# SerezD/vqvae-vqgan-pytorch-lightning

Hardware: AMD Instinct MI355X
Metric: images/sec/node (256x256 bs=32/GPU) VQ-VAE train step (higher is better)
Workload: dtype bf16; 1 GPU; standard_vqvae cb=1024, 256x256 bs=32/GPU (encoder+VQ+decoder fwd/bwd + AdamW); yaml=example_confs/standard_vqvae.yaml, global_batch=32, parallelism=dp1, launch=hipGraph replay (fwd+bwd) + eager all-reduce + AdamW, deterministic=False

## Files before the change

include/vqk.h:

```cpp
#ifndef VQK_H_
#define VQK_H_

#include <stddef.h>
#include <stdint.h>

#ifdef __cplusplus
extern "C" {
#endif

#define VQK_F32 0
#define VQK_BF16 1

enum vqk_status {
    VQK_OK = 0,
    VQK_ERR_SHAPE = -1,
    VQK_ERR_DTYPE = -2,
    VQK_ERR_ALIGN = -3,
    VQK_ERR_LAUNCH = -4,
    VQK_ERR_ARG = -5,
    VQK_ERR_WORKSPACE = -6
};

const char* vqk_status_str(int status);
int vqk_version(void);
// ... 145 lines not shown
                               float scale, const void* zeros, void* stream);
int vqk_conv2d_wgrad_pooled_dy_phase(int dtype, const void* x, const void* dy_pooled, float* dw, int n, int h, int w, int cin,
                                     int cout, float scale, const void* zeros, void* stream);
int vqk_conv2d_wgrad_general(int dtype, const void* x, const void* dy, float* dw, int n, int h_in, int w_in, int cin,
                             int cout, int ksize, int stride, int pad, int mode, int h_out, int w_out,
                             const void* zeros, void* stream);
int vqk_conv2d_fprop_x3_gnstats(const float* x, const void* w5, const float* bias, const float* residual, float* y, int n, int h_in,
                                int w_in, int cin, int cout, int ups, double* gn_ws, int groups, const void* zeros, void* stream);
int vqk_split_pair_f32(const float* src, void* dst, int64_t rows, int c, void* stream);
int vqk_conv2d_wgrad_x3_f32(const float* x, const float* dy, float* dw, int n, int h_in, int w_in, int cin, int cout, int ups,
                            float scale, void* stream);
int vqk_conv2d_wgrad_x3(const void* x_pair, const void* dy_pair, float* dw, int n, int h_in, int w_in, int cin, int cout, int ups,
                        float scale, const void* zeros, void* stream);
int vqk_conv2d_wgrad_general_scaled(int dtype, const void* x, const void* dy, float* dw, int n, int h_in, int w_in, int cin,
                                    int cout, int ksize, int stride, int pad, int mode, int h_out, int w_out, float scale,
                                    const void* zeros, void* stream);
int vqk_conv2d_s2_supported(int dtype, int n, int h_out, int w_out, int cin, int cout, int backward);
int vqk_conv2d_s2_fprop(int dtype, const void* x, const void* wq, const float* bias, void* y, int n, int h_out, int w_out,
                        int cin, int cout, int act, float acc_scale, float out_gain, const void* zeros, void* stream);
int vqk_conv2d_s2_dgrad(int dtype, const void* dy, const void* w3, const void* wt0, void* dx, int n, int h_out, int w_out,
                        int cin, int cout, float acc_scale, const void* zeros, void* stream);
int vqk_conv_weight_layout(int dtype, int n, int h_in, int w_in, int cin, int cout, int ksize, int ups);
int64_t vqk_conv_packed_elems(int cout, int cin, int ksize, int layout);
int vqk_conv_pack_weights(const float* w, void* out, int dtype, int cout, int cin, int ksize, int transpose,
                          int layout, void* stream);
int vqk_conv_pack_multi(const int64_t* descs_dev, int ndesc, int blocks_per_desc, void* stream);
int vqk_conv_set_variant(int variant);
int vqk_conv_fprop_plan(int dtype, int out_dtype, int n, int h_in, int w_in, int cin, int cout, int ksize, int ups, int act,
                        int wlayout, int flags, int* details);
const char* vqk_conv_fprop_form_name(int form, int dtype);
int vqk_set_deterministic(int on, void* ws, int64_t ws_bytes);
int vqk_set_scratch(void* ws, int64_t ws_bytes);
int vqk_set_tile_queue(void* ws, int64_t ws_bytes);
typedef struct vqk_ctx vqk_ctx;
int vqk_ctx_create(vqk_ctx** ctx);
int vqk_ctx_destroy(vqk_ctx* ctx);
int vqk_ctx_make_current(vqk_ctx* ctx);
int vqk_ctx_set_scratch(vqk_ctx* ctx, void* ws, int64_t ws_bytes);
int vqk_ctx_set_tile_queue(vqk_ctx* ctx, void* ws, int64_t ws_bytes);
int vqk_ctx_set_deterministic(vqk_ctx* ctx, int on, void* ws, int64_t ws_bytes);
int vqk_set_tuning(const char* name, int value);
int vqk_reset_tuning(void);
int vqk_tuning_count(void);
const char* vqk_tuning_name(int i);
int vqk_conv_set_block_caps(int stream_blocks, int wgrad_blocks);
int vqk_probe_stream_add(const float* src, float* dst, int64_t bytes, int blocks, int passes, int sleep, void* stream);
int vqk_calib_fill(void* w, int64_t bytes, void* stream);
int vqk_calib_mfma(const void* w, int64_t w_bytes, float* sink, int iters, int blocks, void* stream);
int64_t vqk_calib_mfma_flops(int iters, int blocks);
int vqk_calib_copy(const void* src, void* dst, int64_t bytes, void* stream);
int vqk_conv_pack_dgrad(const float* w, void* wt, int dtype, int cout, int cin, int ksize, void* stream);
int vqk_conv2d_wgrad(int dtype, const void* x, const void* dy, float* dw, int n, int h_in, int w_in, int cin,
                     int cout, int ksize, int ups, const void* zeros, void* stream);
typedef struct vqk_wgrad_item {
    const void* x;
    const void* dy;
    float* dw;
    int dtype, n, h, w, cin, cout, ksize, ups;
    float scale;
    int reserved;
} vqk_wgrad_item;
int vqk_conv3x3_wgrad_group(const vqk_wgrad_item* items, int n_items, const void* zeros, void* stream);
int vqk_conv3x3_wgrad_group_plan(const vqk_wgrad_item* items, int n_items, int* splits, int* launches);
int64_t vqk_conv2d_wgrad_edge_ws_bytes(void);
int vqk_conv2d_wgrad_edge(int dtype, const void* x, const void* dy, float* dw, void* ws, int64_t ws_bytes, int n, int h,
                          int w, int cin, int cout, const void* zeros, void* stream);
int vqk_conv2d_wgrad_edge_true(int dtype, const void* x, const void* dy, float* dw, void* ws, int64_t ws_bytes, int n, int h,
                               int w, int cin, int cout, int thin_true, const void* zeros, void* stream);
int vqk_conv2d_thin_out(int dtype, const void* x, const void* w, const float* bias, void* y, int n, int h, int wd, int cin,
                        int cout, int act, const void* zeros, void* stream);
int vqk_colsum(int dtype, const void* x, int64_t rows, int c, float* out, void* stream);
int vqk_colsum_lead(int dtype, const void* x, int64_t rows, int c, int c_out, float scale, float* out, void* stream);
int vqk_cast(const float* src, void* dst, int dtype, int64_t n, void* stream);

int vqk_gn_stats(int dtype, const void* x, int n, int64_t hw, int c, int groups, float eps,
                 double* acc, float* stats, void* stream);
int vqk_gn_apply(int dtype, const void* x, const float* stats, const float* w, const float* b, void* y,
                 int n, int64_t hw, int c, int groups, int silu, void* stream);
int vqk_gn_forward(int dtype, const void* x, const float* w, const float* b, void* y, float* stats, double* ws, int n,
                   int64_t hw, int c, int groups, float eps, int silu, void* stream);
int vqk_gn_forward_presummed(int dtype, const void* x, const float* w, const float* b, void* y, float* stats, double* ws,
                             int n, int64_t hw, int c, int groups, float eps, int silu, void* stream);
int vqk_gn_forward_presummed_parts(int dtype, const void* x, const float* w, const float* b, void* y, float* stats,
                                   const double* parts, int nblk, double* sums, int n, int64_t hw, int c, int groups, float eps,
                                   int silu, void* stream);
int vqk_gn_backward(int dtype, const void* x, const float* stats, const float* w, const float* b, const void* dy,
                    void* dx, float* dw, float* db, double* red, int n, int64_t hw, int c, int groups, int silu,
                    int accumulate, const void* add, void* stream);
int vqk_gn_backward_ws(int dtype, const void* x, const float* stats, const float* w, const float* b, const void* dy,
                       void* dx, float* dw, float* db, double* red, int64_t ws_doubles, int n, int h, int wd, int c, int groups,
                       int silu, int accumulate, const void* add, const void* add_pooled, float add_scale, void* stream);
int vqk_gn_cluster_timeouts(int* count);
int vqk_gn_backward_colsum(int dtype, const void* x, const float* stats, const float* w, const float* b, const void* dy,
                           void* dx, float* dw, float* db, double* red, int64_t ws_doubles, int n, int h, int wd, int c, int groups,
                           int silu, int accumulate, const void* add, float* dx_colsum, void* stream);
int vqk_gn_backward_pooled_add(int dtype, const void* x, const float* stats, const float* w, const float* b, const void* dy,
                               void* dx, float* dw, float* db, double* red, int n, int h, int wd, int c, int groups, int silu,
                               const void* add_pooled, float add_scale, void* stream);

int vqk_pool2x2(int dtype, const void* x, void* y, int n, int h, int w, int c, float scale, void* stream);
int vqk_unpool2x2(int dtype, const void* x, void* y, int n, int h, int w, int c, float scale, void* stream);
int vqk_preprocess(const float* images, void* x_pad, int dtype, float* target, int n, int h, int w, int cpad,
                   void* stream);
int vqk_augment_preprocess(const float* images, const float* box, const int32_t* flip, void* x_pad, int dtype, float* target,
                           int n, int h, int w, int cpad, void* stream);
int vqk_sse(int dtype, const void* recon, const float* target, int64_t n, float* loss, void* stream);
// ... 124 lines not shown
```

vqvae-vqgan-pytorch-lightning_amd/_native.py:

```python
from __future__ import annotations

import ctypes
import fcntl
import os
import subprocess
from ctypes import c_char_p, c_double, c_float, c_int, c_int32, c_int64, c_void_p, POINTER

_HERE = os.path.dirname(os.path.abspath(__file__))
_CSRC = os.path.join(_HERE, 'csrc')
_SO = os.environ.get('VQK_LIB') or os.path.join(_HERE, 'libvqk.so')
_lib = None

P = c_void_p
I, L, F = c_int, c_int64, c_float


class WgradItem(ctypes.Structure):
    _fields_ = [('x', c_void_p), ('dy', c_void_p), ('dw', c_void_p), ('dtype', c_int), ('n', c_int), ('h', c_int), ('w', c_int),
                ('cin', c_int), ('cout', c_int), ('ksize', c_int), ('ups', c_int), ('scale', c_float), ('reserved', c_int)]


_PROTOS = {
    'vqk_row_sqnorm_f32': [P, L, I, P, P],
    'vqk_vq_assign_f32': [P, P, P, P, L, I, I, I, P, P],
# ... 34 lines not shown
    'vqk_conv4x4_bgrad': [I, P, P, L, I, I, F, I, P, L, P],
    'vqk_bn_forward': [I, P, P, P, P, P, P, P, P, P, L, I, F, F, I, I, P, L, P],
    'vqk_bn_backward': [I, P, P, P, P, P, P, P, P, P, I, L, I, I, P, L, P],
    'vqk_rvq_forward_f32': [P, P, P, L, L, I, I, I, P, P, P, P, P, P],
    'vqk_rvq_decode_f32': [P, P, L, I, I, I, P, P, P],
    'vqk_rvq_backward_f32': [P, P, P, P, I, L, I, I, I, F, F, P, P, P, P, L, P],
    'vqk_l2norm_rows_f32': [P, L, I, P, P, P],
    'vqk_cos_prepare_f32': [P, I, I, P, L, P],
    'vqk_cos_forward_f32': [P, P, L, L, I, I, P, P, P, P, P, P],
    'vqk_cos_sse_f32': [P, P, L, I, P, P],
    'vqk_cos_decode_f32': [P, P, L, L, I, I, P, P, P],
    'vqk_cos_backward_f32': [P, P, P, P, I, L, I, I, F, F, P, P, P, P, L, P],
    'vqk_gvq_forward_f32': [P, P, P, L, I, I, I, P, P, P, P, P, P],
    'vqk_gvq_decode_f32': [P, P, L, I, I, I, P, P, P],
    'vqk_gvq_backward_f32': [P, P, P, P, I, L, I, I, I, F, F, P, P, P, P, L, P],
    'vqk_simvq_project_f32': [P, P, P, I, I, P, P],
    'vqk_simvq_hist_i32': [P, L, I, P, P],
    'vqk_simvq_backward_f32': [P, P, P, P, P, I, L, I, I, F, F, P, P, P, P, P, L, P],
    'vqk_kmeans_seed_step_f32': [P, L, I, I, I, P, P, P, P, P, L, P],
    'vqk_kmeans_update_f32': [P, P, I, I, P, P, P],
    'vqk_ema_stats_f32': [P, P, L, I, I, P, P, P],
    'vqk_ema_stats_fused_f32': [P, P, L, I, I, P, P, P],
    'vqk_ema_update_f32': [P, P, P, P, P, I, I, F, F, F, P],
    'vqk_conv2d_fprop': [I, P, P, P, P, P, I, I, I, I, I, I, I, I, I, I, P, P],
    'vqk_conv2d_fprop_pooled': [I, P, P, P, P, P, I, I, I, I, I, I, I, F, P, P],
    'vqk_conv2d_fprop_gnstats': [I, P, P, P, P, P, I, I, I, I, I, I, I, I, F, P, I, P, P],
    'vqk_conv2d_ups_phase': [I, P, P, P, P, I, I, I, I, I, I, P, I, P, P],
    'vqk_conv2d_pooled_dgrad_phase': [I, P, P, P, I, I, I, I, I, F, P, P],
    'vqk_conv2d_pooled_fprop_phase': [I, P, P, P, P, I, I, I, I, I, F, P, I, P, P],
    'vqk_conv2d_thin_in_gnstats': [I, P, P, P, P, I, I, I, I, P, I, P],
    'vqk_conv2d_s2_supported': [I, I, I, I, I, I, I],
    'vqk_conv2d_s2_fprop': [I, P, P, P, P, I, I, I, I, I, I, F, F, P, P],
    'vqk_conv2d_s2_dgrad': [I, P, P, P, P, I, I, I, I, I, F, P, P],
    'vqk_conv2d_general': [I, P, P, P, P, P, I, I, I, I, I, I, I, I, I, I, I, I, I, F, F, I, P, P],
    'vqk_conv2d_wgrad_general': [I, P, P, P, I, I, I, I, I, I, I, I, I, I, I, P, P],
    'vqk_conv2d_wgrad_general_scaled': [I, P, P, P, I, I, I, I, I, I, I, I, I, I, I, F, P, P],
    'vqk_conv_weight_layout': [I, I, I, I, I, I, I, I],
    'vqk_conv_pack_weights': [P, P, I, I, I, I, I, I, P],
    'vqk_conv_pack_multi': [P, I, I, P],
    'vqk_conv_set_variant': [I],
    'vqk_conv_fprop_plan': [I, I, I, I, I, I, I, I, I, I, I, I, P],
    'vqk_conv_set_block_caps': [I, I],
    'vqk_set_deterministic': [I, P, L],
    'vqk_set_scratch': [P, L],
    'vqk_set_tile_queue': [P, L],
    'vqk_ctx_create': [P],
    'vqk_ctx_destroy': [P],
    'vqk_ctx_make_current': [P],
    'vqk_ctx_set_scratch': [P, P, L],
    'vqk_ctx_set_tile_queue': [P, P, L],
    'vqk_ctx_set_deterministic': [P, I, P, L],
    'vqk_conv_pack_dgrad': [P, P, I, I, I, I, P],
    'vqk_conv2d_wgrad': [I, P, P, P, I, I, I, I, I, I, I, P, P],
    'vqk_conv3x3_wgrad_group': [P, I, P, P],
    'vqk_conv3x3_wgrad_group_plan': [P, I, P, P],
    'vqk_conv2d_wgrad_pooled_dy': [I, P, P, P, I, I, I, I, I, F, P, P],
    'vqk_conv2d_wgrad_ups_phase': [I, P, P, P, I, I, I, I, I, F, P, P],
    'vqk_split_pair_f32': [P, P, L, I, P],
    'vqk_conv2d_fprop_x3_gnstats': [P, P, P, P, P, I, I, I, I, I, I, P, I, P, P],
    'vqk_conv2d_wgrad_x3': [P, P, P, I, I, I, I, I, I, F, P, P],
    'vqk_conv2d_wgrad_x3_f32': [P, P, P, I, I, I, I, I, I, F, P],
    'vqk_conv2d_wgrad_pooled_dy_phase': [I, P, P, P, I, I, I, I, I, F, P, P],
    'vqk_conv2d_wgrad_edge': [I, P, P, P, P, L, I, I, I, I, I, P, P],
    'vqk_conv2d_wgrad_edge_true': [I, P, P, P, P, L, I, I, I, I, I, I, P, P],
    'vqk_conv2d_thin_out': [I, P, P, P, P, I, I, I, I, I, I, P, P],
    'vqk_colsum': [I, P, L, I, P, P],
    'vqk_colsum_lead': [I, P, L, I, I, F, P, P],
    'vqk_cast': [P, P, I, L, P],
    'vqk_gn_stats': [I, P, I, L, I, I, F, P, P, P],
    'vqk_gn_apply': [I, P, P, P, P, P, I, L, I, I, I, P],
    'vqk_gn_forward': [I, P, P, P, P, P, P, I, L, I, I, F, I, P],
    'vqk_gn_forward_presummed': [I, P, P, P, P, P, P, I, L, I, I, F, I, P],
    'vqk_gn_forward_presummed_parts': [I, P, P, P, P, P, P, I, P, I, L, I, I, F, I, P],
    'vqk_gn_backward': [I, P, P, P, P, P, P, P, P, P, I, L, I, I, I, I, P, P],
    'vqk_gn_backward_pooled_add': [I, P, P, P, P, P, P, P, P, P, I, I, I, I, I, I, P, F, P],
    'vqk_gn_backward_ws': [I, P, P, P, P, P, P, P, P, P, L, I, I, I, I, I, I, I, P, P, F, P],
    'vqk_gn_cluster_timeouts': [P],
    'vqk_gn_backward_colsum': [I, P, P, P, P, P, P, P, P, P, L, I, I, I, I, I, I, I, P, P, P],
    'vqk_pool2x2': [I, P, P, I, I, I, I, F, P],
    'vqk_unpool2x2': [I, P, P, I, I, I, I, F, P],
    'vqk_preprocess': [P, P, I, P, I, I, I, I, P],
    'vqk_augment_preprocess': [P, P, P, P, I, P, I, I, I, I, P],
    'vqk_sse': [I, P, P, L, P, P],
    'vqk_pair_stats': [P, P, L, P, P],
    'vqk_ssim_sum': [P, P, I, I, I, I, P, I, P, F, F, P, P],
    'vqk_mse_tanh_backward': [I, P, P, L, F, P, I, P, P],
    'vqk_tanh_backward': [I, P, P, P, L, P],
    'vqk_axpby': [I, P, P, P, F, F, L, P],
    'vqk_adamw': [P, P, P, P, L, P, P, I, F, F, F, F, I, F, P, P],
    'vqk_step_guard': [P, I, c_double, F, F, P, L, P, P, P],
    'vqk_adamw_guarded': [P, P, P, P, L, P, P, I, F, F, F, F, P, P, P],
    'vqk_act_backward': [I, P, P, P, L, I, F, P],
    'vqk_act_backward_colsum': [I, P, P, P, L, I, I, F, P, P],
    'vqk_act_backward_colsum_scaled': [I, P, P, P, L, I, I, F, F, P, P],
    'vqk_upfirdn2d_nhwc': [I, P, P, P, I, I, I, I, I, I, I, I, I, I, I, I, I, I, I, F, I, I, P],
    'vqk_upfirdn2d_act_backward': [I, P, P, P, P, I, I, I, I, I, I, I, I, I, F, I, I, I, P],
    'vqk_maxpool2x2': [I, P, P, P, I, I, I, I, I, P],
    'vqk_channel_affine': [I, P, P, P, P, L, I, P],
    'vqk_lpips_tap': [I, P, P, P, I, L, I, P, P, F, P, P],
    'vqk_mbstd': [I, P, P, P, P, I, L, I, I, I, I, P],
    'vqk_mbstd_double_backward': [I, P, P, P, P, P, I, L, I, I, I, P],
    'vqk_l1_sum': [I, P, P, L, P, P],
    'vqk_l1l2_backward': [I, P, P, L, F, F, P, P, I, P],
    'vqk_gan_loss': [P, P, I, I, I, P, P, P, P, P],
    'vqk_bias_act': [P, P, P, P, P, P, L, L, I, I, I, F, F, F, P],
    'vqk_upfirdn2d': [P, P, P, I, I, I, I, I, I, I, I, I, I, I, I, I, I, I, F, I, I, P],
# ... 97 lines not shown
```

vqvae-vqgan-pytorch-lightning_amd/csrc/api.cpp:

```cpp
#include <stdint.h>
#include <new>
#include "common.h"

extern "C" {

const char* vqk_status_str(int status) {
    switch (status) {
        case VQK_OK: return "ok";
        case VQK_ERR_SHAPE: return "unsupported or inconsistent shape";
        case VQK_ERR_DTYPE: return "unsupported dtype";
        case VQK_ERR_ALIGN: return "pointer is not 16-byte aligned";
        case VQK_ERR_LAUNCH: return "kernel launch failed";
        case VQK_ERR_ARG: return "bad argument";
        case VQK_ERR_WORKSPACE: return "workspace too small";
        default: return "unknown status";
    }
}

int vqk_version(void) { return 1; }
const char* vqk_arch(void) { return "gfx950"; }

}

struct vqk_ctx {
// ... 61 lines not shown
    d.on = on ? 1 : 0;
    d.ws = (on && ws) ? reinterpret_cast<float*>(ws) : nullptr;
    d.bytes = (on && ws) ? ws_bytes : 0;
    return VQK_OK;
}

extern "C" int vqk_set_tile_queue(void* ws, int64_t ws_bytes) { return vqk_ctx_set_tile_queue(nullptr, ws, ws_bytes); }
extern "C" int vqk_set_scratch(void* ws, int64_t ws_bytes) { return vqk_ctx_set_scratch(nullptr, ws, ws_bytes); }
extern "C" int vqk_set_deterministic(int on, void* ws, int64_t ws_bytes) { return vqk_ctx_set_deterministic(nullptr, on, ws, ws_bytes); }

#include <string.h>
#include <stdlib.h>
namespace vqkd {
static TuneSlot g_tune[] = {
    {"MX", 0, 0},
    {"MX_1X1", 0, 0},
    {"TW16", 0, 0},
    {"STREAM_BLOCKS", 0, 0},
    {"MX_MIN_TILES", 0, 0},
    {"FPROP_SPLITK", 0, 0},
    {"SK_BLOCKS", 0, 0},
    {"SK_MINSTEPS", 0, 0},
    {"SK_MAXMB", 0, 0},
    {"UPS_PHASE", 0, 0},
    {"WGRAD_BLOCKS", 0, 0},
    {"WGMX", 0, 0},
    {"WGRAD_GEN_BLOCKS", 0, 0},
    {"WGRAD_NO_PW16", 0, 0},
    {"WGRAD_NO_P16K", 0, 0},
    {"MX_HALF", 0, 0},
    {"MX_HALF_HW", 0, 0},
    {"UPFIRDN_TILE", 0, 0},
    {"GN_BLOCKS_REDUCE", 0, 0},
    {"GN_BLOCKS_APPLY", 0, 0},
    {"GN_NT_MB", 0, 0},
    {"GN_NO_SMALL", 0, 0},
    {"WGMX_COEF_E4", 0, 0},
    {"GN_CLUSTER_MAX_HW", 0, 0},
    {"COMM_CUS", 0, 0},
    {"MX_QUARTER", 0, 0},
    {"MX_S2", 0, 0},
    {"MX_S2_DGRAD_MIN", 0, 0},
    {"VQ_LDS", 0, 0},
    {"UPS_MERGE", 0, 0},
    {"TILE_QUEUE", 0, 0},
    {"X3_WL", 0, 0},
    {"X3_WGRAD_COEF_E4", 0, 0},
    {"X3_WGRAD_FOLD", 0, 0},
    {"X3_WGRAD_PHASE", 0, 0},
    {"X3_WGRAD_PHASE_CAP_PCT", 0, 0},
    {"X3_WGRAD_PHASE_COEF_E4", 0, 0},
    {"WGRAD_GROUP_LOAD_PCT", 0, 0},
    {"WGRAD_GROUP_MIN_PPS", 0, 0},
    {"MX_PHASE_U64", 0, 0}
};
static constexpr int kTune = (int)(sizeof(g_tune) / sizeof(g_tune[0]));
TuneSlot* tune_slot(const char* name) {
    for (int i = 0; i < kTune; ++i)
        if (strcmp(g_tune[i].name, name) == 0) return &g_tune[i];
    abort();
}
}

extern "C" int vqk_set_tuning(const char* name, int value) {
    if (!name) return VQK_ERR_ARG;
    for (int i = 0; i < vqkd::kTune; ++i)
        if (strcmp(vqkd::g_tune[i].name, name) == 0) {
            __atomic_store_n(&vqkd::g_tune[i].value, value, __ATOMIC_RELAXED);
            __atomic_store_n(&vqkd::g_tune[i].is_set, 1, __ATOMIC_RELEASE);
            return VQK_OK;
        }
    return VQK_ERR_ARG;
}

extern "C" int vqk_reset_tuning(void) {
    for (int i = 0; i < vqkd::kTune; ++i) __atomic_store_n(&vqkd::g_tune[i].is_set, 0, __ATOMIC_RELAXED);
    return VQK_OK;
}

extern "C" int vqk_tuning_count(void) { return vqkd::kTune; }

extern "C" const char* vqk_tuning_name(int i) { return (i >= 0 && i < vqkd::kTune) ? vqkd::g_tune[i].name : nullptr; }
```

vqvae-vqgan-pytorch-lightning_amd/ops.py:

```python
from __future__ import annotations

import ctypes
import os
import threading
import weakref

import numpy as _np
import torch

from . import _native

F32, BF16 = 0, 1
_CL = torch.channels_last


def dcode(dtype: torch.dtype) -> int:
    if dtype == torch.float32:
        return F32
    if dtype == torch.bfloat16:
        return BF16
    raise RuntimeError(f'vqk: unsupported dtype {dtype}')


def epc(dtype: torch.dtype) -> int:
# ... 771 lines not shown
        torch.zeros((cout, ksize, ksize, cin), dtype=torch.float32, device=x.device).permute(0, 3, 1, 2)
    flops = 2.0 * n * dy.shape[2] * dy.shape[3] * cout * cin * ksize * ksize
    if edge_wgrad_served(x, dy, ksize, ups):
        ws = _edge_ws(x.device)
        nbytes = (x.numel() + dy.numel()) * 2
        st = _timed('conv3x3_wgrad_thin_kernel<bf16>' + (f' {cin}->{cout}@{h}x{w}' if _EVENT_SHAPES else ''), 0.0,
                    lambda: _native.lib().vqk_conv2d_wgrad_edge_true(dcode(x.dtype), x.data_ptr(), dy.data_ptr(), dw.data_ptr(),
                                                                     ws.data_ptr(), ws.numel() * 4, n, h, w, cin, cout, int(thin_true),
                                                                     zero_page(x.device).data_ptr(), _stream()), nbytes)
        _native.check(st, 'conv2d_wgrad_edge')
        return dw
    if thin_true != 8:
        raise RuntimeError('vqk: an unpadded weight-gradient target needs the edge-conv kernel')
    if (x3 and not X3_WGRAD_FOLD and x.dtype == torch.float32 and dy.dtype == torch.float32 and ksize == 3 and cin % 64 == 0
            and cout % 64 == 0 and dy.shape[3] % 8 == 0 and dy.shape[2] % 8 == 0 and not DETERMINISTIC):
        phase = bool(ups) and X3_WGRAD_PHASE and h % 8 == 0 and w % 8 == 0
        st = _timed('conv3x3_wgrad_x3_kernel<f32 as 3 x bf16>' + (f' {cin}->{cout}@{dy.shape[2]}x{dy.shape[3]} k3{" phase" if phase else ""}' if _EVENT_SHAPES else ''), flops,
                    lambda: _native.lib().vqk_conv2d_wgrad_x3_f32(x.data_ptr(), dy.data_ptr(), dw.data_ptr(), n, h, w, cin, cout, int(ups),
                                                                  1.0, _stream()), exec_flops=3.0 * flops * (4.0 / 9.0 if phase else 1.0))
        if st != _native.ERR_SHAPE:
            _native.check(st, 'conv2d_wgrad_x3_f32')
            return dw
    if (x3 and x.dtype == torch.float32 and dy.dtype == torch.float32 and ksize == 3 and cin % 64 == 0 and cout % 64 == 0
            and dy.shape[3] % 16 == 0 and dy.shape[2] % 8 == 0 and not DETERMINISTIC and _WGMX_ON):
        xp, dyp = raw_split_pair(x), raw_split_pair(dy)
        st = _timed('conv3x3_wgrad_mx_kernel<f32 as 3 x bf16>' + (f' {cin}->{cout}@{dy.shape[2]}x{dy.shape[3]} k3' if _EVENT_SHAPES else ''), flops,
                    lambda: _native.lib().vqk_conv2d_wgrad_x3(xp.data_ptr(), dyp.data_ptr(), dw.data_ptr(), n, h, w, cin, cout, int(ups),
                                                              1.0, zero_page(x.device).data_ptr(), _stream()), exec_flops=3.0 * flops)
        if st != _native.ERR_SHAPE:
            _native.check(st, 'conv2d_wgrad_x3')
            return dw
    if (ups and UPS_PHASE_WGRAD and _WGMX_ON and x.dtype == torch.bfloat16 and ksize == 3 and cin % 64 == 0 and cout % 64 == 0
            and w % 16 == 0 and h % 8 == 0 and not DETERMINISTIC):
        st = _timed('conv3x3_wgrad_mx_kernel<bf16>' + (f' {cin}->{cout}@{dy.shape[2]}x{dy.shape[3]} k{ksize} phase' if _EVENT_SHAPES else ''), flops,
                    lambda: _native.lib().vqk_conv2d_wgrad_ups_phase(dcode(x.dtype), x.data_ptr(), dy.data_ptr(), dw.data_ptr(), n, h, w,
                                                                     cin, cout, 1.0, zero_page(x.device).data_ptr(), _stream()),
                    launches=4, exec_flops=flops * 4.0 / 9.0)
        if st != _native.ERR_SHAPE:
            _native.check(st, 'conv2d_wgrad_ups_phase')
            return dw
    mxw = (_WGMX_ON and x.dtype == torch.bfloat16 and ksize == 3 and cin % 64 == 0 and cout % 64 == 0
           and dy.shape[3] % 16 == 0 and dy.shape[2] % 8 == 0)
    kname = 'conv3x3_wgrad_mx_kernel<bf16>' if mxw else f'conv_wgrad_kernel<{"f32" if x.dtype == torch.float32 else "bf16"}>'
    if _EVENT_SHAPES:
        kname += f' {cin}->{cout}@{dy.shape[2]}x{dy.shape[3]} k{ksize}'
    st = _timed(kname, flops,
                lambda: _native.lib().vqk_conv2d_wgrad(dcode(x.dtype), x.data_ptr(), dy.data_ptr(), dw.data_ptr(), n, h,
                                                       w, cin, cout, ksize, int(ups),
                                                       zero_page(x.device).data_ptr(), _stream()))
    _native.check(st, 'conv2d_wgrad')
    return dw


X3_WGRAD_PHASE = _native.switch('VQK_X3_WGRAD_PHASE', '1') != '0'


def raw_conv_wgrad_pooled_x3(x, dy_pooled, scale: float, out) -> bool:
    n, cin, h, w = x.shape
    cout = dy_pooled.shape[1]
    if (not X3_WGRAD_PHASE or x.dtype != torch.float32 or dy_pooled.dtype != torch.float32 or cin % 64 or cout % 64 or h % 16 or w % 16
            or DETERMINISTIC or tuple(dy_pooled.shape[2:]) != (h // 2, w // 2)):
        return False
    flops = 2.0 * n * h * w * cout * cin * 9
    st = _timed('conv3x3_wgrad_x3_kernel<f32 as 3 x bf16>' + (f' {cin}->{cout}@{h}x{w} k3 pooled-dy phase' if _EVENT_SHAPES else ''), flops,
                lambda: _native.lib().vqk_conv2d_wgrad_x3_f32(x.data_ptr(), dy_pooled.data_ptr(), out.data_ptr(), n, h, w, cin, cout, 2,
                                                              float(scale), _stream()), exec_flops=3.0 * flops * 4.0 / 9.0)
    if st == _native.ERR_SHAPE:
        return False
    _native.check(st, 'conv2d_wgrad_x3_f32')
    return True


def raw_conv_wgrad_pooled_dy(x, dy_pooled, scale: float, out) -> bool:
    n, cin, h, w = x.shape
    cout = dy_pooled.shape[1]
    if not (_WGMX_ON and x.dtype == torch.bfloat16 and cin % 64 == 0 and cout % 64 == 0 and w % 16 == 0 and h % 8 == 0):
        return False
    flops = 2.0 * n * h * w * cout * cin * 9
    if POOLED_WGRAD_PHASE and not DETERMINISTIC and (h // 2) % 8 == 0 and (w // 2) % 16 == 0:
        st = _timed('conv3x3_wgrad_mx_kernel<bf16>' + (f' {cin}->{cout}@{h}x{w} pooled-dy phase' if _EVENT_SHAPES else ''), flops,
                    lambda: _native.lib().vqk_conv2d_wgrad_pooled_dy_phase(dcode(x.dtype), x.data_ptr(), dy_pooled.data_ptr(), out.data_ptr(),
                                                                           n, h // 2, w // 2, cin, cout, float(scale),
                                                                           zero_page(x.device).data_ptr(), _stream()),
                    exec_flops=flops * 4.0 / 9.0)
        if st != _native.ERR_SHAPE:
            _native.check(st, 'conv2d_wgrad_pooled_dy_phase')
            return True
    st = _timed('conv3x3_wgrad_mx_kernel<bf16>' + (f' {cin}->{cout}@{h}x{w} pooled-dy' if _EVENT_SHAPES else ''), flops,
                lambda: _native.lib().vqk_conv2d_wgrad_pooled_dy(dcode(x.dtype), x.data_ptr(), dy_pooled.data_ptr(), out.data_ptr(),
                                                                 n, h, w, cin, cout, float(scale),
                                                                 zero_page(x.device).data_ptr(), _stream()))
    if st == _native.ERR_SHAPE:
        return False
    _native.check(st, 'conv2d_wgrad_pooled_dy')
    return True


def raw_colsum(x2d_rows: int, c: int, x, out=None, lead: int | None = None, scale: float = 1.0) -> torch.Tensor:
    out = out if out is not None else torch.zeros(c, dtype=torch.float32, device=x.device)
    _native.check(_native.lib().vqk_colsum_lead(dcode(x.dtype), x.data_ptr(), x2d_rows, c, c if lead is None else lead, float(scale),
                                                out.data_ptr(), _stream()), 'colsum')
    return out


def raw_cast(src_f32, dtype) -> torch.Tensor:
    if dtype == torch.float32:
# ... 828 lines not shown
        t1, t2 = direct_grad(c1w), direct_grad(c2w)
        tw1, tb1, tw2, tb2 = direct_grad(n1w), direct_grad(n1b), direct_grad(n2w), direct_grad(n2b)
        if (pool and POOLED_BWD and scw is None and dt == torch.bfloat16 and t1 is not None and t2 is not None
                and None not in (tw1, tb1, tw2, tb2) and OVERLAP_WGRAD and h * w > 1024 and cout % 128 == 0 and w % 16 == 0 and h % 8 == 0
                and weight_layout(dt, n, h // 2, w // 2, cout, cout, 3, True) == 1 and _MX_ON and _WGMX_ON):
            main, side = torch.cuda.current_stream(), _side_stream(x.device)
            lib = _native.lib()
            lib.vqk_conv_set_block_caps(OVERLAP_STREAM_BLOCKS, _wgrad_cap(h * w))
            try:
                lay = weight_layout(dt, n, h // 2, w // 2, cout, cout, 3, True)
                wt2 = packed_weight(c2w, cout, cout, dt, 3, True, lay)
                d_a2 = raw_conv_pooled_dgrad_phase(dout, c2w, 0.25) if POOLED_DGRAD_PHASE else None
                if d_a2 is None:
                    d_a2 = _conv_general_raw(dout, wt2, None, None, cout, 3, 1, 1, 1, h, w, 0, 0.25, 1.0, dt, lay)

                def wgrad2_pooled():
                    if not raw_conv_wgrad_pooled_dy(a2, dout, 0.25, t2):
                        raise RuntimeError('vqk: pooled weight gradient not served for an eligible shape')
                _on_side(main, side, wgrad2_pooled)
                d_r1, _, _ = raw_gn_backward(r1, st2, w2, b2, d_a2, groups, True, tw2, tb2, cluster_ok=ctx.cluster_ok)
                main.wait_stream(side)
                lay1 = weight_layout(dt, n, h, w, cout, cin, 3, False)
                d_a1 = raw_conv_fprop(d_r1, packed_weight(c1w, cin, cout, dt, 3, True, lay1), None, None, 3, False, 0, dt, cin, lay1)
                _on_side(main, side, lambda: raw_conv_wgrad(a1, d_r1, 3, False, out=t1, x3=x3))
                dx = raw_gn_backward_pooled_add(x, st1, w1, b1, d_a1, groups, True, tw1, tb1, dout, 0.25, cluster_ok=ctx.cluster_ok)
                main.wait_stream(side)
            finally:
                lib.vqk_conv_set_block_caps(0, 0)
            return dx, None, None, None, None, None, None, None, None, None, None, None
        d_a2_pre = dout_p = None
        if pool:
            if x3 and POOLED_DGRAD_PHASE and h % 16 == 0 and w % 32 == 0:
                d_a2_pre = raw_conv_pooled_dgrad_phase(dout, c2w, 0.25, x3=True)
            dout_p = dout if x3 else None
            dout = raw_unpool(dout, 0.25)

        def wgrad_c2(tgt):
            if dout_p is not None and raw_conv_wgrad_pooled_x3(a2, dout_p, 0.25, tgt):
                return
            raw_conv_wgrad(a2, dout, 3, False, out=tgt, x3=x3)

        def conv_bwd(inp, dy, wparam, k, ci, co, need_dx=True, need_dw=True):
            dx = None
            if need_dx:
                lay = weight_layout(dt, n, h, w, co, ci, k, False, x3=x3)
                wt = packed_weight(wparam, ci, co, dt, k, True, lay)
                dx = raw_conv_fprop(dy, wt, None, None, k, False, 0, dt, ci, lay)
            if not need_dw:
                return dx, None
            tgt = direct_grad(wparam)
            dw = raw_conv_wgrad(inp, dy, k, False, out=tgt, x3=x3)
            return dx, (None if tgt is not None else dw)

        def gn_bwd(inp, st, wv, bv, dy, wparam, bparam, add=None, colsum_of=None):
            tw, tb = direct_grad(wparam), direct_grad(bparam)
            direct = tw is not None and tb is not None
            cs = None
            if colsum_of is not None and gn_colsum_ok(h, w) and not torch.is_grad_enabled():
                cs = direct_grad(colsum_of)
                if cs is not None:
                    _DB_DONE.add(id(colsum_of))
            dx, dw, db = raw_gn_backward(inp, st, wv, bv, dy, groups, True, tw if direct else None,
                                         tb if direct else None, add=add, dx_colsum=cs, cluster_ok=ctx.cluster_ok)
            if direct:
                return dx, None, None
            return dx, dw.view(wparam.shape), db.view(bparam.shape)

        if OVERLAP_WGRAD and t1 is not None and t2 is not None:
            main, side = torch.cuda.current_stream(), _side_stream(x.device)
            lib = _native.lib()
            lib.vqk_conv_set_block_caps(OVERLAP_STREAM_BLOCKS, _wgrad_cap(h * w))
            try:
                d_a2 = d_a2_pre if d_a2_pre is not None else conv_bwd(a2, dout, c2w, 3, cout, cout, need_dw=False)[0]
                group = dout_p is None and wgrad_group_deferrable(a2, dout, t2, x3) and wgrad_group_deferrable(a1, dout, t1, x3)
                if group:
                    defer_wgrad(a2, dout, t2)
                else:
                    _on_side(main, side, lambda: wgrad_c2(t2))
                d_r1, dn2w, dn2b = gn_bwd(r1, st2, w2, b2, d_a2, n2w, n2b)
                if not group:
                    main.wait_stream(side)
                d_a1, _ = conv_bwd(a1, d_r1, c1w, 3, cin, cout, need_dw=False)
                if group:
                    defer_wgrad(a1, d_r1, t1)
                else:
                    _on_side(main, side, lambda: raw_conv_wgrad(a1, d_r1, 3, False, out=t1, x3=x3))
                dskip, dwsc = dout, None
                if scw is not None:
                    dskip, dwsc = conv_bwd(x, dout, scw, 1, cin, cout)
                dx, dn1w, dn1b = gn_bwd(x, st1, w1, b1, d_a1, n1w, n1b, add=dskip, colsum_of=ctx.db_param)
                if not group:
                    main.wait_stream(side)
            finally:
                lib.vqk_conv_set_block_caps(0, 0)
            return dx, dn1w, dn1b, None, dn2w, dn2b, None, dwsc, None, None, None, None
        d_a2, dw2 = conv_bwd(a2, dout, c2w, 3, cout, cout, need_dx=d_a2_pre is None)
        if d_a2_pre is not None:
            d_a2 = d_a2_pre
        d_r1, dn2w, dn2b = gn_bwd(r1, st2, w2, b2, d_a2, n2w, n2b)
        d_a1, dw1 = conv_bwd(a1, d_r1, c1w, 3, cin, cout)
        dskip, dwsc = dout, None
        if scw is not None:
            dskip, dwsc = conv_bwd(x, dout, scw, 1, cin, cout)
        dx, dn1w, dn1b = gn_bwd(x, st1, w1, b1, d_a1, n1w, n1b, add=dskip, colsum_of=ctx.db_param)
        return dx, dn1w, dn1b, dw1, dn2w, dn2b, dw2, dwsc, None, None, None, None


def res_block(x, n1w, n1b, c1w, n2w, n2b, c2w, scw=None, groups: int = 32, eps: float = 1e-6, pool: bool = False,
              next_gn: int = 0):
    return ResBlockFn.apply(x, n1w, n1b, c1w, n2w, n2b, c2w, scw, groups, eps, pool, next_gn)


def group_norm_silu(x, weight, bias, groups: int = 32, eps: float = 1e-6, silu: bool = True):
    return GroupNormSiLUFn.apply(x, weight, bias, groups, eps, silu)


class AvgPool2x2Fn(torch.autograd.Function):

    @staticmethod
    def forward(ctx, x):
        _require_gpu(x)
        return raw_pool(nhwc(x), 0.25)

    @staticmethod
    def backward(ctx, dy):
        return raw_unpool(nhwc(dy), 0.25)


def avg_pool2x2(x):
    return AvgPool2x2Fn.apply(x)


def mse_loss(recon, target, true_channels: int | None = None):
    n, c, h, w = recon.shape
    return _MSE.apply(recon, target, float(n * (true_channels or c) * h * w))


class _MSE(torch.autograd.Function):
    @staticmethod
    def forward(ctx, recon, target, denom: float):
        _require_gpu(recon)
        recon = nhwc(recon)
        target = nhwc(target.to(torch.float32))
        if recon.shape != target.shape:
            raise RuntimeError(f'vqk: mse shapes differ {tuple(recon.shape)} vs {tuple(target.shape)}')
        sse = torch.zeros((), dtype=torch.float32, device=recon.device)
        _native.check(_native.lib().vqk_sse(dcode(recon.dtype), recon.data_ptr(), target.data_ptr(), recon.numel(),
                                            sse.data_ptr(), _stream()), 'sse')
        ctx.save_for_backward(recon, target)
        ctx.denom = denom
        return sse / denom

    @staticmethod
    def backward(ctx, dloss):
        recon, target = ctx.saved_tensors
        d = torch.empty_like(recon, memory_format=_CL)
# ... 84 lines not shown
```

Baseline: 1184 images/sec.

## Fuse 1x1 shortcut conv dgrad and wgrad into one streaming kernel

Adds a HIP kernel that computes both dx and dw of the 1x1 residual shortcut conv in a single pass over pixels. Each block stages dy and x tiles in LDS and runs MFMA for both products, accumulating dw in registers and flushing it with atomics. Block start points are staggered so the atomic flushes are spread out. This replaces two separate kernels that each read dy and is meant to cut memory traffic and launch overhead. The cost is non-deterministic atomic accumulation of dw and a new code path limited to particular shapes.

```diff
diff --git a/include/vqk.h b/include/vqk.h
--- a/include/vqk.h
+++ b/include/vqk.h
@@ -221,6 +221,8 @@
 int vqk_conv_pack_dgrad(const float* w, void* wt, int dtype, int cout, int cin, int ksize, void* stream);
 int vqk_conv2d_wgrad(int dtype, const void* x, const void* dy, float* dw, int n, int h_in, int w_in, int cin,
                      int cout, int ksize, int ups, const void* zeros, void* stream);
+int vqk_conv1x1_bwd(int dtype, const void* x, const void* dy, const float* w, void* dx, float* dw, int n, int h, int wd, int cin,
+                    int cout, void* stream);
 typedef struct vqk_wgrad_item {
     const void* x;
     const void* dy;
diff --git a/vqvae-vqgan-pytorch-lightning_amd/_native.py b/vqvae-vqgan-pytorch-lightning_amd/_native.py
--- a/vqvae-vqgan-pytorch-lightning_amd/_native.py
+++ b/vqvae-vqgan-pytorch-lightning_amd/_native.py
@@ -110,6 +110,7 @@
     'vqk_ctx_set_deterministic': [P, I, P, L],
     'vqk_conv_pack_dgrad': [P, P, I, I, I, I, P],
     'vqk_conv2d_wgrad': [I, P, P, P, I, I, I, I, I, I, I, P, P],
+    'vqk_conv1x1_bwd': [I, P, P, P, P, P, I, I, I, I, I, P],
     'vqk_conv3x3_wgrad_group': [P, I, P, P],
     'vqk_conv3x3_wgrad_group_plan': [P, I, P, P],
     'vqk_conv2d_wgrad_pooled_dy': [I, P, P, P, I, I, I, I, I, F, P, P],
diff --git a/vqvae-vqgan-pytorch-lightning_amd/csrc/api.cpp b/vqvae-vqgan-pytorch-lightning_amd/csrc/api.cpp
--- a/vqvae-vqgan-pytorch-lightning_amd/csrc/api.cpp
+++ b/vqvae-vqgan-pytorch-lightning_amd/csrc/api.cpp
@@ -137,7 +137,11 @@
     {"X3_WGRAD_PHASE_COEF_E4", 0, 0},
     {"WGRAD_GROUP_LOAD_PCT", 0, 0},
     {"WGRAD_GROUP_MIN_PPS", 0, 0},
-    {"MX_PHASE_U64", 0, 0}
+    {"MX_PHASE_U64", 0, 0},
+    {"CONV1X1_BWD", 0, 0},
+    {"CONV1X1_BWD_BLOCKS", 0, 0},
+    {"CONV1X1_BWD_MIN_STEPS", 0, 0},
+    {"CONV1X1_BWD_STAGGER_PCT", 0, 0}
 };
 static constexpr int kTune = (int)(sizeof(g_tune) / sizeof(g_tune[0]));
 TuneSlot* tune_slot(const char* name) {
diff --git a/vqvae-vqgan-pytorch-lightning_amd/csrc/conv1x1_bwd.hip b/vqvae-vqgan-pytorch-lightning_amd/csrc/conv1x1_bwd.hip
--- /dev/null
+++ b/vqvae-vqgan-pytorch-lightning_amd/csrc/conv1x1_bwd.hip
@@ -0,0 +1,278 @@
+#include "conv_geom.h"
+
+namespace {
+
+constexpr int C1_PS = 64;
+constexpr int C1_PAD = 16;
+constexpr int C1_MAX_ACC = 32768;
+constexpr int C1_MAX_SLICE = 256;
+constexpr int C1_LDS_MAX = 160 * 1024;
+
+typedef bf16x8_t frag_t;
+
+__device__ __forceinline__ frag_t c1_tr_frag(const char* p, int stride) {
+    const s16x4 lo = __builtin_amdgcn_ds_read_tr16_b64_v4i16((VQK_LDS s16x4*)p);
+    const s16x4 hi = __builtin_amdgcn_ds_read_tr16_b64_v4i16((VQK_LDS s16x4*)(p + 4 * stride));
+    typedef __attribute__((ext_vector_type(8))) short s16x8;
+    const s16x8 v = {lo[0], lo[1], lo[2], lo[3], hi[0], hi[1], hi[2], hi[3]};
+    return __builtin_bit_cast(frag_t, v);
+}
+
+struct C1Args {
+    const bf16_raw* x; const bf16_raw* dy; const float* w; bf16_raw* dx; float* dw;
+    int pixels, cin, cout, slice, steps, stagger_pct;
+};
+
+__host__ __device__ inline int c1_first_step(int64_t b, int64_t nb, int64_t steps, int64_t p) {
+    return (int)(steps * ((100 - p) * b * nb + p * b * b) / (100 * nb * nb));
+}
+
+__host__ __device__ constexpr int c1_lds_bytes_pad(int cout, int slice, int padx) {
+    return cout * (slice * 2 + padx) + C1_PS * (cout * 2 + C1_PAD) + C1_PS * (slice * 2 + padx) + C1_PS * (slice * 2 + C1_PAD);
+}
+__host__ __device__ constexpr int c1_padx(int cout, int slice) {
+    return c1_lds_bytes_pad(cout, slice, 64) <= C1_LDS_MAX ? 64 : C1_PAD;
+}
+__host__ __device__ constexpr int c1_lds_bytes(int cout, int slice) { return c1_lds_bytes_pad(cout, slice, c1_padx(cout, slice)); }
+
+template <int CO, int SL>
+__global__ __launch_bounds__(512) void conv1x1_bwd_kernel(const C1Args a) {
+    extern __shared__ __attribute__((aligned(16))) char smem[];
+    constexpr bool FIXED = CO > 0;
+    const int tid = threadIdx.x, lane = tid & 63;
+    const int wave = __builtin_amdgcn_readfirstlane(tid >> 6);
+    const int s_begin = c1_first_step(blockIdx.x, gridDim.x, a.steps, a.stagger_pct);
+    const int s_end = c1_first_step(blockIdx.x + 1, gridDim.x, a.steps, a.stagger_pct);
+    if (s_begin >= s_end) return;
+    const int co_n = FIXED ? CO : a.cout, sl_n = FIXED ? SL : a.slice, cin = a.cin;
+    const int ci0 = (int)blockIdx.y * sl_n;
+    const int SD = co_n * 2 + C1_PAD, SX = sl_n * 2 + c1_padx(co_n, sl_n), SO = sl_n * 2 + C1_PAD;
+    char* const wl = smem;
+    char* const dyl = wl + co_n * SX;
+    char* const xl = dyl + C1_PS * SD;
+    char* const dxl = xl + C1_PS * SX;
+    auto barrier = [&]() { asm volatile("s_waitcnt lgkmcnt(0)\n\ts_barrier" ::: "memory"); };
+
+    const int ndy = co_n >> 6, nx = sl_n >> 6;
+    const int dy_ppr = co_n >> 3, x_ppr = sl_n >> 3;
+    int dyl_off[8], xl_off[4], ol_off[4], xg_off[4], x_row[4];
+#pragma unroll
+    for (int i = 0; i < 8; ++i) {
+        const int q = tid + 512 * i, row = q / dy_ppr;
+        dyl_off[i] = q * 16 + row * C1_PAD;
+    }
+#pragma unroll
+    for (int i = 0; i < 4; ++i) {
+        const int q = tid + 512 * i, row = q / x_ppr, col = q - row * x_ppr;
+        x_row[i] = row;
+        xl_off[i] = row * SX + col * 16;
+        ol_off[i] = row * SO + col * 16;
+        xg_off[i] = ci0 + col * 8;
+    }
+    constexpr int DEPTH = (FIXED && CO <= 256) ? 2 : 1;
+    struct Rows { vqk_u32x4 dy[8], x[4]; };
+    Rows ring[DEPTH];
+    auto load_step = [&](int s, Rows& rw) {
+        const int64_t p0 = (int64_t)s * C1_PS;
+        const int rows = (int)min((int64_t)C1_PS, (int64_t)a.pixels - p0);
+        const bf16_raw* dyb = a.dy + p0 * co_n;
+        const int lim = rows * co_n - 8;
+#pragma unroll
+        for (int i = 0; i < 8; ++i)
+            if (i < ndy) rw.dy[i] = *reinterpret_cast<const vqk_u32x4*>(dyb + min((tid + 512 * i) * 8, lim));
+#pragma unroll
+        for (int i = 0; i < 4; ++i)
+            if (i < nx) rw.x[i] = *reinterpret_cast<const vqk_u32x4*>(a.x + (p0 + min(x_row[i], rows - 1)) * cin + xg_off[i]);
+    };
+    auto stage_step = [&](int s, const Rows& rw) {
+        const int rows = (int)min((int64_t)C1_PS, (int64_t)a.pixels - (int64_t)s * C1_PS);
+        const int lim = rows * co_n;
+        const vqk_u32x4 zero = {0u, 0u, 0u, 0u};
+#pragma unroll
+        for (int i = 0; i < 8; ++i)
+            if (i < ndy) *reinterpret_cast<vqk_u32x4*>(dyl + dyl_off[i]) = (tid + 512 * i) * 8 < lim ? rw.dy[i] : zero;
+#pragma unroll
+        for (int i = 0; i < 4; ++i)
+            if (i < nx) *reinterpret_cast<vqk_u32x4*>(xl + xl_off[i]) = rw.x[i];
+    };
+
+    load_step(s_begin, ring[0]);
+    if (DEPTH == 2 && s_begin + 1 < s_end) load_step(s_begin + 1, ring[DEPTH - 1]);
+    {
+        const int qpr = sl_n >> 2, total = co_n * qpr;
+        for (int q = tid; q < total; q += 512) {
+            const int co = q / qpr, c4 = q - co * qpr;
+            const f32x4 v = *reinterpret_cast<const f32x4*>(a.w + (int64_t)co * cin + ci0 + c4 * 4);
+            typedef __attribute__((ext_vector_type(2))) unsigned int u32x2;
+            const u32x2 o = {(unsigned)f32_to_bf16(v[0]) | ((unsigned)f32_to_bf16(v[1]) << 16),
+                             (unsigned)f32_to_bf16(v[2]) | ((unsigned)f32_to_bf16(v[3]) << 16)};
+            *reinterpret_cast<u32x2*>(wl + co * SX + c4 * 8) = o;
+        }
+    }
+
+    const int li = lane & 15, grp = (lane >> 4) & 1, kgrp = lane >> 5;
+    const int tr_dy = ((li >> 2) + 8 * kgrp) * SD + (16 * grp + 4 * (li & 3)) * 2;
+    const int tr_x = ((li >> 2) + 8 * kgrp) * SX + (16 * grp + 4 * (li & 3)) * 2;
+    const int nci = sl_n >> 6;
+    const bool dw_wave = wave < (co_n >> 6) * nci;
+    const int tco = wave / nci, tci = wave - tco * nci;
+    const int dx_tiles = 2 * (sl_n >> 5);
+    f32x16 acc[2][2];
+#pragma unroll
+    for (int i = 0; i < 2; ++i)
+#pragma unroll
+        for (int j = 0; j < 2; ++j)
+#pragma unroll
+            for (int r = 0; r < 16; ++r) acc[i][j][r] = 0.0f;
+
+    auto dw_step = [&]() {
+        if (!dw_wave) return;
+        const char* pa = dyl + tr_dy + tco * 128;
+        const char* pb = xl + tr_x + tci * 128;
+#pragma unroll
+        for (int kb = 0; kb < C1_PS / 16; ++kb) {
+            const frag_t a0 = c1_tr_frag(pa + kb * 16 * SD, SD), a1 = c1_tr_frag(pa + kb * 16 * SD + 64, SD);
+            const frag_t b0 = c1_tr_frag(pb + kb * 16 * SX, SX), b1 = c1_tr_frag(pb + kb * 16 * SX + 64, SX);
+            acc[0][0] = __builtin_amdgcn_mfma_f32_32x32x16_bf16(a0, b0, acc[0][0], 0, 0, 0);
+            acc[0][1] = __builtin_amdgcn_mfma_f32_32x32x16_bf16(a0, b1, acc[0][1], 0, 0, 0);
+            acc[1][0] = __builtin_amdgcn_mfma_f32_32x32x16_bf16(a1, b0, acc[1][0], 0, 0, 0);
+            acc[1][1] = __builtin_amdgcn_mfma_f32_32x32x16_bf16(a1, b1, acc[1][1], 0, 0, 0);
+        }
+    };
+    auto dx_tile = [&](int t) {
+        const int tp = t & 1, tc = t >> 1;
+        const char* pw = wl + tr_x + tc * 64;
+        const char* pd = dyl + (tp * 32 + (lane & 31)) * SD + kgrp * 16;
+        f32x16 d;
+#pragma unroll
+        for (int r = 0; r < 16; ++r) d[r] = 0.0f;
+        if constexpr (FIXED) {
+#pragma unroll
+            for (int kb = 0; kb < CO / 16; ++kb) {
+                const frag_t wf = c1_tr_frag(pw + kb * 16 * SX, SX);
+                const frag_t df = *reinterpret_cast<const frag_t*>(pd + kb * 32);
+                d = __builtin_amdgcn_mfma_f32_32x32x16_bf16(wf, df, d, 0, 0, 0);
+            }
+        } else {
+            for (int kb = 0; kb < (co_n >> 4); ++kb) {
+                const frag_t wf = c1_tr_frag(pw + kb * 16 * SX, SX);
+                const frag_t df = *reinterpret_cast<const frag_t*>(pd + kb * 32);
+                d = __builtin_amdgcn_mfma_f32_32x32x16_bf16(wf, df, d, 0, 0, 0);
+            }
+        }
+        char* po = dxl + (tp * 32 + (lane & 31)) * SO + (tc * 32 + 4 * kgrp) * 2;
+#pragma unroll
+        for (int rq = 0; rq < 4; ++rq) {
+            typedef __attribute__((ext_vector_type(2))) unsigned int u32x2;
+            const u32x2 o = {vqk_pack_bf16x2(d[4 * rq], d[4 * rq + 1]), vqk_pack_bf16x2(d[4 * rq + 2], d[4 * rq + 3])};
+            *reinterpret_cast<u32x2*>(po + rq * 16) = o;
+        }
+    };
+    auto dx_step = [&]() {
+        for (int t = wave; t < dx_tiles; t += 8) dx_tile(t);
+    };
+    const bool dx_first = (wave >> 2) & 1;
+
+    auto step = [&](int s, Rows& rw) {
+        stage_step(s, rw);
+        barrier();
+        if (s + DEPTH < s_end) load_step(s + DEPTH, rw);
+        if (dx_first) { dx_step(); dw_step(); }
+        else { dw_step(); dx_step(); }
+        barrier();
+        const int64_t p0 = (int64_t)s * C1_PS;
+        const int rows = (int)min((int64_t)C1_PS, (int64_t)a.pixels - p0);
+#pragma unroll
+        for (int i = 0; i < 4; ++i)
+            if (i < nx && x_row[i] < rows)
+                *reinterpret_cast<vqk_u32x4*>(a.dx + (p0 + x_row[i]) * cin + xg_off[i]) =
+                    *reinterpret_cast<const vqk_u32x4*>(dxl + ol_off[i]);
+    };
+    for (int s = s_begin; s < s_end; s += DEPTH) {
+        step(s, ring[0]);
+        if (DEPTH == 2 && s + 1 < s_end) step(s + 1, ring[DEPTH - 1]);
+    }
+
+    if (dw_wave) {
+#pragma unroll
+        for (int i = 0; i < 2; ++i)
+#pragma unroll
+            for (int j = 0; j < 2; ++j) {
+                const int ci = ci0 + tci * 64 + j * 32 + (lane & 31);
+#pragma unroll
+                for (int r = 0; r < 16; ++r) {
+                    const int co = tco * 64 + i * 32 + (r & 3) + 8 * (r >> 2) + 4 * kgrp;
+                    atomicAdd(a.dw + (int64_t)co * cin + ci, acc[i][j][r]);
+                }
+            }
+    }
+}
+
+int c1_slice(int cin, int cout) {
+    for (int sl = cin < C1_MAX_SLICE ? cin : C1_MAX_SLICE; sl >= 64; sl -= 64)
+        if (cin % sl == 0 && (int64_t)cout * sl <= C1_MAX_ACC && c1_lds_bytes(cout, sl) <= C1_LDS_MAX) return sl;
+    return 0;
+}
+
+template <int CO, int SL>
+int c1_launch(const C1Args& a, int blocks, int slices, hipStream_t st) {
+    static const hipError_t attr = hipFuncSetAttribute((const void*)conv1x1_bwd_kernel<CO, SL>, hipFuncAttributeMaxDynamicSharedMemorySize, C1_LDS_MAX);
+    if (attr != hipSuccess) return VQK_ERR_LAUNCH;
+    hipLaunchKernelGGL((conv1x1_bwd_kernel<CO, SL>), dim3((unsigned)blocks, (unsigned)slices), dim3(512), c1_lds_bytes(a.cout, a.slice), st, a);
+    VQK_CHECK_LAUNCH();
+    return VQK_OK;
+}
+
+}
+
+namespace vqkd {
+
+bool conv1x1_bwd_serves(int dtype, int64_t pixels, int cin, int cout) {
+    return dtype == VQK_BF16 && VQK_TUNE("CONV1X1_BWD", 1) != 0 && !det_state().on && conv_force_variant() == CONV_VARIANT_AUTO
+        && pixels >= 1 && cin >= 64 && cout >= 64 && (cin % 64) == 0 && (cout % 64) == 0 && c1_slice(cin, cout) > 0
+        && pixels * (cin > cout ? cin : cout) < (1ll << 30);
+}
+
+}
+
+extern "C" int vqk_conv1x1_bwd(int dtype, const void* x, const void* dy, const float* w, void* dx, float* dw, int n, int h, int wd,
+                               int cin, int cout, void* stream) {
+    VQK_REQUIRE(dtype == VQK_F32 || dtype == VQK_BF16, VQK_ERR_DTYPE);
+    VQK_REQUIRE(n >= 1 && h >= 1 && wd >= 1 && cin >= 1 && cout >= 1, VQK_ERR_SHAPE);
+    const int64_t pixels = (int64_t)n * h * wd;
+    VQK_REQUIRE(vqkd::conv1x1_bwd_serves(dtype, pixels, cin, cout), VQK_ERR_SHAPE);
+    VQK_REQUIRE(x && dy && w && dx && dw, VQK_ERR_ARG);
+    VQK_REQUIRE(vqk_aligned16(x) && vqk_aligned16(dy) && vqk_aligned16(w) && vqk_aligned16(dx) && vqk_aligned16(dw), VQK_ERR_ALIGN);
+    C1Args a;
+    a.x = (const bf16_raw*)x; a.dy = (const bf16_raw*)dy; a.w = w; a.dx = (bf16_raw*)dx; a.dw = dw;
+    a.pixels = (int)pixels; a.cin = cin; a.cout = cout; a.slice = c1_slice(cin, cout);
+    a.steps = (int)((pixels + C1_PS - 1) / C1_PS);
+    const int slices = cin / a.slice;
+    int blocks = VQK_TUNE("CONV1X1_BWD_BLOCKS", 0);
+    if (blocks <= 0) {
+        const int min_steps = VQK_TUNE("CONV1X1_BWD_MIN_STEPS", 4);
+        VQK_REQUIRE(min_steps >= 1, VQK_ERR_ARG);
+        blocks = 256 / slices;
+        if ((int64_t)blocks * min_steps > a.steps) blocks = (a.steps + min_steps - 1) / min_steps;
+    }
+    VQK_REQUIRE(blocks <= 4096, VQK_ERR_ARG);
+    if (blocks < 1) blocks = 1;
+    int pct = VQK_TUNE("CONV1X1_BWD_STAGGER_PCT", -1);
+    if (pct < 0) {
+        const double t_atomic = (double)blocks * slices * cout * a.slice * 4.0 / 1.3e12;
+        const double t_stream = (double)pixels * (cout + 2.0 * cin) * 2.0 / 5.0e12;
+        pct = (int)(100.0 * t_atomic / (2.0 * t_stream));
+    }
+    a.stagger_pct = pct > 50 ? 50 : pct;
+    hipStream_t st = vqk_stream(stream);
+    const int key = cout * 1024 + a.slice;
+    switch (key) {
+        case 64 * 1024 + 64: return c1_launch<64, 64>(a, blocks, slices, st);
+        case 128 * 1024 + 64: return c1_launch<128, 64>(a, blocks, slices, st);
+        case 128 * 1024 + 128: return c1_launch<128, 128>(a, blocks, slices, st);
+        case 128 * 1024 + 256: return c1_launch<128, 256>(a, blocks, slices, st);
+        case 256 * 1024 + 128: return c1_launch<256, 128>(a, blocks, slices, st);
+        case 512 * 1024 + 64: return c1_launch<512, 64>(a, blocks, slices, st);
+        default: return c1_launch<0, 0>(a, blocks, slices, st);
+    }
+}
diff --git a/vqvae-vqgan-pytorch-lightning_amd/ops.py b/vqvae-vqgan-pytorch-lightning_amd/ops.py
--- a/vqvae-vqgan-pytorch-lightning_amd/ops.py
+++ b/vqvae-vqgan-pytorch-lightning_amd/ops.py
@@ -847,6 +847,30 @@
     return dw
 
 
+CONV1X1_BWD = _native.switch('VQK_CONV1X1_BWD', '1') != '0'
+
+
+def raw_conv1x1_bwd(x, dy, weight, tgt):
+    n, cin, h, w = x.shape
+    cout = dy.shape[1]
+    wd = weight.detach()
+    if (not CONV1X1_BWD or DETERMINISTIC or x.dtype != torch.bfloat16 or dy.dtype != torch.bfloat16 or tgt is None
+            or wd.dtype != torch.float32 or tgt.dtype != torch.float32 or tuple(wd.shape) != (cout, cin, 1, 1)
+            or tuple(tgt.shape) != (cout, cin, 1, 1) or not wd.is_contiguous() or not tgt.is_contiguous()
+            or tuple(dy.shape) != (n, cout, h, w)):
+        return None
+    dx = empty_nhwc(n, cin, h, w, x.dtype, x.device)
+    pix = n * h * w
+    st = _timed('conv1x1_bwd_kernel<bf16>' + (f' {cin}->{cout}@{h}x{w} k1 dx+dw' if _EVENT_SHAPES else ''), 4.0 * pix * cin * cout,
+                lambda: _native.lib().vqk_conv1x1_bwd(dcode(x.dtype), x.data_ptr(), dy.data_ptr(), wd.data_ptr(), dx.data_ptr(),
+                                                      tgt.data_ptr(), n, h, w, cin, cout, _stream()),
+                pix * (cout + 2 * cin) * 2.0 + cout * cin * 12.0)
+    if st == _native.ERR_SHAPE:
+        return None
+    _native.check(st, 'conv1x1_bwd')
+    return dx
+
+
 X3_WGRAD_PHASE = _native.switch('VQK_X3_WGRAD_PHASE', '1') != '0'
 
 
@@ -1781,6 +1805,13 @@
             dw = raw_conv_wgrad(inp, dy, k, False, out=tgt, x3=x3)
             return dx, (None if tgt is not None else dw)
 
+        def shortcut_bwd():
+            if not x3:
+                dskip = raw_conv1x1_bwd(x, dout, scw, direct_grad(scw))
+                if dskip is not None:
+                    return dskip, None
+            return conv_bwd(x, dout, scw, 1, cin, cout)
+
         def gn_bwd(inp, st, wv, bv, dy, wparam, bparam, add=None, colsum_of=None):
             tw, tb = direct_grad(wparam), direct_grad(bparam)
             direct = tw is not None and tb is not None
@@ -1816,7 +1847,7 @@
                     _on_side(main, side, lambda: raw_conv_wgrad(a1, d_r1, 3, False, out=t1, x3=x3))
                 dskip, dwsc = dout, None
                 if scw is not None:
-                    dskip, dwsc = conv_bwd(x, dout, scw, 1, cin, cout)
+                    dskip, dwsc = shortcut_bwd()
                 dx, dn1w, dn1b = gn_bwd(x, st1, w1, b1, d_a1, n1w, n1b, add=dskip, colsum_of=ctx.db_param)
                 if not group:
                     main.wait_stream(side)
@@ -1830,7 +1861,7 @@
         d_a1, dw1 = conv_bwd(a1, d_r1, c1w, 3, cin, cout)
         dskip, dwsc = dout, None
         if scw is not None:
-            dskip, dwsc = conv_bwd(x, dout, scw, 1, cin, cout)
+            dskip, dwsc = shortcut_bwd()
         dx, dn1w, dn1b = gn_bwd(x, st1, w1, b1, d_a1, n1w, n1b, add=dskip, colsum_of=ctx.db_param)
         return dx, dn1w, dn1b, dw1, dn2w, dn2b, dw2, dwsc, None, None, None, None
 
```

Result: no change. 1189 images/sec (median of 6 runs) (+0.4%).
